# takurot/Pyrope

Hardware: NVIDIA B200
Metric: batched VEC.SEARCH QPS at fixed recall@10 (higher is better)
Workload: dtype f32 LUT / u8 codes

## Files before the change

### pyrope_b200/csrc/pq_lm.cu

```cuda
#include <cub/cub.cuh>

#include <cstdio>
#include <type_traits>

#include "common.cuh"
#include "exact_arith.cuh"
#include "kernels.h"

namespace pyrope {
namespace {

constexpr int LM_SCAN_WARPS = 8;
constexpr int LM_BUILD_WARPS = 8;
constexpr int LM_THREADS = 32 * (LM_SCAN_WARPS + LM_BUILD_WARPS);
constexpr int LM_BLK_STAGES = 6;
constexpr int LM_QS = 8;
constexpr int LM_QC = 256;
constexpr int LM_PF = 4;
constexpr int LM_HDR = 96;
constexpr int LM_MAX_DIM = 128;
constexpr int LM_LUT_BYTES = 256 * 256;
constexpr int LM_BLK_MAX = LM_HDR + LM_MAX_DIM * 32;
constexpr int LM_QSETS = 3;
constexpr int LM_SMEM = 2 * LM_LUT_BYTES + LM_BLK_STAGES * LM_BLK_MAX + LM_QSETS * LM_QS * LM_QC * 8;
constexpr float LM_QMAX = 2046.f;
constexpr float LM_QERR = 8.25f;
constexpr int LM_HB = 64;
constexpr int SEED_NQ = 2;
constexpr int SEED_CAP = 1024;
constexpr int REDO_QCAP = 2048;

struct __align__(16) LmHeader {
    int list, nvec;
    long long vbeg;
    int qid[LM_QS];
    short pslot[LM_QS];
    float s[LM_QS];
};
static_assert(LM_BUILD_WARPS == LM_QS && LM_SCAN_WARPS % 4 == 0, "one builder warp per query slot; builders start a TMEM lane quadrant");
static_assert(sizeof(LmHeader) == LM_HDR, "header size");

__device__ __forceinline__ uint32_t smem_u32(const void* p) { return (uint32_t)__cvta_generic_to_shared(p); }
__device__ __forceinline__ bool elect_one() {
    uint32_t pred;
    asm volatile("{\n\t.reg .pred p;\n\telect.sync _|p, 0xffffffff;\n\tselp.u32 %0, 1, 0, p;\n\t}" : "=r"(pred));
    return pred != 0;
}
__device__ __forceinline__ void mbar_init(uint32_t bar, uint32_t count) {
    asm volatile("mbarrier.init.shared::cta.b64 [%0], %1;" ::"r"(bar), "r"(count));
}
__device__ __forceinline__ void mbar_expect_tx(uint32_t bar, uint32_t bytes) {
    asm volatile("mbarrier.arrive.expect_tx.shared::cta.b64 _, [%0], %1;" ::"r"(bar), "r"(bytes) : "memory");
}
__device__ __forceinline__ bool mbar_try_wait(uint32_t bar, uint32_t parity) {
// ... 22 lines not shown
__device__ __forceinline__ void bulk_g2s(uint32_t dst, const void* src, uint32_t bytes, uint32_t bar) {
    asm volatile("cp.async.bulk.shared::cluster.global.mbarrier::complete_tx::bytes [%0], [%1], %2, [%3];"
                 ::"r"(dst), "l"(src), "r"(bytes), "r"(bar)
                 : "memory");
}
__device__ __forceinline__ unsigned long long pack2(float a, float b) {
    unsigned long long d;
    asm("mov.b64 %0, {%1, %2};" : "=l"(d) : "f"(a), "f"(b));
    return d;
}
__device__ __forceinline__ unsigned long long ffma2(unsigned long long a, unsigned long long b, unsigned long long c) {
    unsigned long long d;
    asm("fma.rn.f32x2 %0, %1, %2, %3;" : "=l"(d) : "l"(a), "l"(b), "l"(c));
    return d;
}



template <int N>
__device__ __forceinline__ void tmem_st(uint32_t taddr, const uint32_t (&r)[N]) {
    static_assert(N == 4 || N == 8, "4 or 8 columns");
    if (N == 8)
        asm volatile("tcgen05.st.sync.aligned.32x32b.x8.b32 [%0], {%1, %2, %3, %4, %5, %6, %7, %8};"
                     ::"r"(taddr), "r"(r[0]), "r"(r[1]), "r"(r[2]), "r"(r[3]), "r"(r[4 % N]), "r"(r[5 % N]), "r"(r[6 % N]), "r"(r[7 % N])
                     : "memory");
    else
        asm volatile("tcgen05.st.sync.aligned.32x32b.x4.b32 [%0], {%1, %2, %3, %4};"
                     ::"r"(taddr), "r"(r[0]), "r"(r[1]), "r"(r[2]), "r"(r[3])
                     : "memory");
}
template <int N>
__device__ __forceinline__ void tmem_ld(uint32_t taddr, uint32_t (&r)[N]) {
    if (N == 8)
        asm volatile("tcgen05.ld.sync.aligned.32x32b.x8.b32 {%0, %1, %2, %3, %4, %5, %6, %7}, [%8];"
                     : "=r"(r[0]), "=r"(r[1]), "=r"(r[2]), "=r"(r[3]), "=r"(r[4 % N]), "=r"(r[5 % N]), "=r"(r[6 % N]), "=r"(r[7 % N])
                     : "r"(taddr)
                     : "memory");
    else
        asm volatile("tcgen05.ld.sync.aligned.32x32b.x4.b32 {%0, %1, %2, %3}, [%4];"
                     : "=r"(r[0]), "=r"(r[1]), "=r"(r[2]), "=r"(r[3])
                     : "r"(taddr)
                     : "memory");
}
__device__ __forceinline__ void tmem_ld_wait() { asm volatile("tcgen05.wait::ld.sync.aligned;" ::: "memory"); }

struct LmParams {
    int dim, ksub, k;
    const float* codebook; const uint8_t* codes; const uint8_t* dead;
    const unsigned char* iblk; const int32_t* n_items;
    unsigned long long* pool; int32_t* pool_cnt; uint32_t* pool_thr; int pslots;
    int kc;
    uint32_t* hist;
    const float* thr0;
    const uint32_t* sinv_max;
    int2* redo; int32_t* redo_cnt;
    int32_t* item_ctr;
    const unsigned long long* thr_pub;
    unsigned long long* peer_thr[7];
    int n_peers;
// ... 76 lines not shown
    for (int w = (int)(((int64_t)blockIdx.x * blockDim.x + threadIdx.x) >> 5); w < n_items; w += wstride) {
        const int l = a.item_list[w], rel = w - a.ioff[l];
        const int64_t beg = a.list_off[l], len = a.list_off[l + 1] - beg;
        const int g = rel;
        const int pbeg = a.loff[l], pend = a.loff[l + 1];
        int qid[LM_QS], psl[LM_QS];
    #pragma unroll
        for (int j = 0; j < LM_QS; ++j) {
            const int idx = pbeg + LM_QS * g + j;
            qid[j] = idx < pend ? a.pairq[idx] : -1;
            psl[j] = idx < pend ? a.pairp[idx] : 0;
        }
        unsigned char* blkp = a.iblk + (size_t)w * a.blk;
        const int sub = a.dim >> 4, D0 = lane * 4;
        const bool on = lane * 4 < a.dim;
        const float cm = on ? __ldg(a.cmax + D0 / sub) : 0.f;
        float4 c = make_float4(0.f, 0.f, 0.f, 0.f);
        if (on) c = __ldg(reinterpret_cast<const float4*>(a.centroids + (size_t)l * a.dim) + lane);
        float scale[LM_QS];
    #pragma unroll
        for (int h = 0; h < LM_QS / 4; ++h) {
            float4 t[4];
    #pragma unroll
            for (int j = 0; j < 4; ++j) {
                float4 q = c;
                if (on && qid[4 * h + j] >= 0) q = __ldg(reinterpret_cast<const float4*>(a.Q + (size_t)qid[4 * h + j] * a.dim) + lane);
                t[j] = make_float4(-2.f * (q.x - c.x), -2.f * (q.y - c.y), -2.f * (q.z - c.z), -2.f * (q.w - c.w));
                float r2 = 0.25f * (t[j].x * t[j].x + t[j].y * t[j].y + t[j].z * t[j].z + t[j].w * t[j].w);
                if (sub == 8) r2 += __shfl_xor_sync(0xffffffffu, r2, 1);
                float b = on ? sqrtf(r2) * 1.000001f + cm : 0.f;
                b *= b;
    #pragma unroll
                for (int o = 16; o > 0; o >>= 1) b = fmaxf(b, __shfl_xor_sync(0xffffffffu, b, o));
                scale[4 * h + j] = qid[4 * h + j] >= 0 ? LM_QMAX / (b * 1.00001f + 1e-30f) : 0.f;
            }
            if (on) {
                float4* dst = reinterpret_cast<float4*>(blkp + LM_HDR + (size_t)h * a.dim * 16);
                dst[((D0 + 0) % sub) * 16 + (D0 + 0) / sub] = make_float4(t[0].x, t[1].x, t[2].x, t[3].x);
                dst[((D0 + 1) % sub) * 16 + (D0 + 1) / sub] = make_float4(t[0].y, t[1].y, t[2].y, t[3].y);
                dst[((D0 + 2) % sub) * 16 + (D0 + 2) / sub] = make_float4(t[0].z, t[1].z, t[2].z, t[3].z);
                dst[((D0 + 3) % sub) * 16 + (D0 + 3) / sub] = make_float4(t[0].w, t[1].w, t[2].w, t[3].w);
            }
        }
        if (lane == 0) {
            LmHeader h{};
            h.list = l;
            h.vbeg = beg;
            h.nvec = (int)len;
    #pragma unroll
            for (int j = 0; j < LM_QS; ++j) { h.qid[j] = qid[j]; h.pslot[j] = (short)psl[j]; h.s[j] = scale[j]; }
            *reinterpret_cast<LmHeader*>(blkp) = h;
        }
        if (lane < LM_QS) {
            float mys = 0.f;
            int myq = -1;
    #pragma unroll
// ... 133 lines not shown
            }
            if (lane == 0) {
                const float t = __uint_as_float(hi);
                const float tp = t + 2e-5f * t + 1e-5f * s_rr[warp] + 1e-12f;
                a.pool_thr[q0 + warp] = score_to_ord(-tp) - 1u;
                a.thr0[q0 + warp] = tp;
            }
        }
    }
}

template <int SUB>
__global__ void __launch_bounds__(LM_THREADS, 1) ivfpq_lm_scan_kernel(LmParams p) {
    extern __shared__ __align__(1024) unsigned char smem[];
    unsigned char* lut0 = smem;
    unsigned char* rbuf = lut0 + 2 * LM_LUT_BYTES;
    uint64_t* qkeys = reinterpret_cast<uint64_t*>(rbuf + LM_BLK_STAGES * LM_BLK_MAX);
    __shared__ __align__(8) uint64_t s_mbar[LM_BLK_STAGES + 4];
    __shared__ int s_qcnt[LM_QSETS * LM_QS];
    __shared__ int s_ti[LM_SCAN_WARPS * LM_QS];
    __shared__ float s_inv[LM_SCAN_WARPS * LM_QS];
    __shared__ uint32_t s_tmem;

    const int tid = threadIdx.x, lane = tid & 31, warp = tid >> 5;
    const bool builder = warp >= LM_SCAN_WARPS;
    const int K = p.ksub;
    const int blk = LM_HDR + p.dim * 32;
    const int n_items = *p.n_items;
    __shared__ int s_item[LM_BLK_STAGES];

    const uint32_t bar_blk = smem_u32(&s_mbar[0]);
    const uint32_t bar_full = smem_u32(&s_mbar[LM_BLK_STAGES]);
    const uint32_t bar_done = smem_u32(&s_mbar[LM_BLK_STAGES + 2]);
    if (tid == 0) {
        for (int i = 0; i < LM_BLK_STAGES; ++i) mbar_init(bar_blk + 8 * i, 1);
        for (int i = 0; i < 2; ++i) { mbar_init(bar_full + 8 * i, LM_BUILD_WARPS); mbar_init(bar_done + 8 * i, LM_SCAN_WARPS); }
        asm volatile("fence.mbarrier_init.release.cluster;" ::: "memory");
    }
    if (tid < LM_QSETS * LM_QS) s_qcnt[tid] = 0;
    for (int i = tid; i < 2 * LM_LUT_BYTES / 16; i += LM_THREADS) reinterpret_cast<uint4*>(lut0)[i] = make_uint4(0u, 0u, 0u, 0u);

    constexpr int BT = LM_BUILD_WARPS * 32;
    constexpr int EPT = 256 * 16 / BT;
    constexpr int TCOLS = (BT / 128) * EPT * SUB;
    if (warp == LM_SCAN_WARPS) {
        asm volatile("tcgen05.alloc.cta_group::1.sync.aligned.shared::cta.b32 [%0], %1;" ::"r"(smem_u32(&s_tmem)), "n"(TCOLS) : "memory");
        asm volatile("tcgen05.relinquish_alloc_permit.cta_group::1.sync.aligned;" ::: "memory");
    }
    asm volatile("tcgen05.fence::before_thread_sync;" ::: "memory");
    __syncthreads();
    asm volatile("tcgen05.fence::after_thread_sync;" ::: "memory");

    auto claim_block = [&](int i) -> bool {
        const uint32_t br = bar_blk + 8 * (i % LM_BLK_STAGES);
        const int g = atomicAdd(p.item_ctr, 1);
        if (g < n_items) {
            s_item[i % LM_BLK_STAGES] = g;
            mbar_expect_tx(br, (uint32_t)blk);
            bulk_g2s(smem_u32(rbuf + (i % LM_BLK_STAGES) * LM_BLK_MAX), p.iblk + (size_t)g * blk, (uint32_t)blk, br);
            return true;
        }
        s_item[i % LM_BLK_STAGES] = -1;
        mbar_arrive(br);
        return false;
    };

    if (builder) {
        const int bw = warp - LM_SCAN_WARPS;
        const int m = lane & 15;
        const int eb = (lane >> 4) + 2 * bw;
        const uint32_t tcb = s_tmem + ((uint32_t)((warp & 3) * 32) << 16) + (uint32_t)((bw >> 2) * EPT * SUB);
        float pn[EPT];
#pragma unroll
        for (int j = 0; j < EPT; ++j) {
            const int e = eb + (BT / 16) * j;
            float s = 0.f;
            uint32_t r[SUB];
#pragma unroll
            for (int d4 = 0; d4 < SUB / 4; ++d4) {
                float4 v = make_float4(0.f, 0.f, 0.f, 0.f);
                if (e < K) v = __ldg(reinterpret_cast<const float4*>(p.codebook + ((size_t)m * K + e) * SUB) + d4);
                r[4 * d4 + 0] = __float_as_uint(v.x); r[4 * d4 + 1] = __float_as_uint(v.y);
                r[4 * d4 + 2] = __float_as_uint(v.z); r[4 * d4 + 3] = __float_as_uint(v.w);
                s = fmaf(v.x, v.x, s); s = fmaf(v.y, v.y, s); s = fmaf(v.z, v.z, s); s = fmaf(v.w, v.w, s);
            }
            tmem_st<SUB>(tcb + j * SUB, r);
            pn[j] = s;
        }
        asm volatile("tcgen05.wait::st.sync.aligned;" ::: "memory");
        bool more = false;
        const bool claimer = bw == 0 && elect_one();
        if (claimer) more = claim_block(0);
        auto tighten = [&](int q, uint32_t ord) {
            if (p.n_peers == 0) {
                atomicMax(p.pool_thr + q, ord);
            } else if (atomicMax(p.pool_thr + q, ord) < ord) {
                const unsigned long long w = ((unsigned long long)p.epoch << 32) | ord;
                for (int r = 0; r < p.n_peers; ++r) atomicMax(p.peer_thr[r] + q, w);
            }
        };
        auto finalize = [&](const LmHeader* hd, int gitem, uint64_t* qk, int* qcnt) {
            const int j = bw;
            int* cntp = &qcnt[j];
            const int n = *cntp;
            const int q = hd->qid[j];
            if (n > 0 && q >= 0) {
                uint64_t* kq = qk + j * LM_QC;
                bool redo = n > LM_QC;
                if (!redo) {
                    const size_t ps = (size_t)q * p.pslots + hd->pslot[j];
                    unsigned long long* dst = p.pool + ps * p.kc;
                    const float err = LM_QERR / hd->s[j];
                    int kept = n;
                    float dk = 0.f;
                    if (n > p.k) {
                        const int P2 = next_pow2(n);
// ... 41 lines not shown
                                const int fl = __ffs(reach) - 1;
                                if (lane == fl) {
                                    const int bk = 2 * lane + ((cum - cc.y >= (uint32_t)p.k) ? 0 : 1);
                                    const float edge = bk == LM_HB - 1 ? t0 * 1.01f + 2.f * err : lo + wid * (float)(bk + 1);
                                    const float errq = LM_QERR * 1.001f * __uint_as_float(__ldg(p.sinv_max + q));
                                    tighten(q, score_to_ord(-(edge * 1.00001f + errq)) - 1u);
                                }
                            }
                        }
                    }
                }
                if (redo && lane == 0) p.redo[atomicAdd(p.redo_cnt, 1)] = make_int2(q, gitem * LM_QS + j);
            }
            __syncwarp();
            if (lane == 0) *cntp = 0;
        };

        auto wait_done = [&](int i) { mbar_wait(bar_done + 8 * (i & 1), (uint32_t)(i >> 1) & 1u); };
        auto hand_over = [&](int i) {
            finalize(reinterpret_cast<const LmHeader*>(rbuf + (i % LM_BLK_STAGES) * LM_BLK_MAX), s_item[i % LM_BLK_STAGES],
                     qkeys + (i % LM_QSETS) * (LM_QS * LM_QC), s_qcnt + (i % LM_QSETS) * LM_QS);
        };
        const unsigned long long magic2 = pack2(8388608.f, 8388608.f);
        const unsigned long long quarter = pack2(0.25f, 0.25f);
        int i = 0;
        for (;; ++i) {
            const int b = i & 1;
            if (i >= 2) wait_done(i - 2);
            if (more) more = claim_block(i + 1);
            mbar_wait(bar_blk + 8 * (i % LM_BLK_STAGES), (uint32_t)(i / LM_BLK_STAGES) & 1u);
            if (s_item[i % LM_BLK_STAGES] < 0) break;
            const unsigned char* blkp = rbuf + (i % LM_BLK_STAGES) * LM_BLK_MAX;
            const LmHeader* hd = reinterpret_cast<const LmHeader*>(blkp);
            if (claimer && hd->nvec > 0)
                bulk_prefetch_l2(p.codes + (size_t)hd->vbeg * 16, (uint32_t)hd->nvec * 16u);
            unsigned char* lut = lut0 + b * LM_LUT_BYTES;
#pragma unroll 1
            for (int h = 0; h < LM_QS / 4; ++h) {
                if (hd->qid[4 * h] < 0) continue;
                const ulonglong2* rt = reinterpret_cast<const ulonglong2*>(blkp + LM_HDR) + h * p.dim + m;
                unsigned long long t01[SUB], t23[SUB], rr01 = 0ull, rr23 = 0ull;
#pragma unroll
                for (int d = 0; d < SUB; ++d) {
                    const ulonglong2 v = rt[d * 16];
                    t01[d] = v.x; t23[d] = v.y;
                    rr01 = ffma2(v.x, v.x, rr01);
                    rr23 = ffma2(v.y, v.y, rr23);
                }
                const float4 sh4 = *reinterpret_cast<const float4*>(hd->s + 4 * h);
                const unsigned long long s01 = pack2(sh4.x, sh4.y), s23 = pack2(sh4.z, sh4.w);
                const bool compact = hd->qid[LM_QS / 2] < 0;
                unsigned char* lw = compact ? lut + eb * 128 + m * 8 : lut + eb * 256 + m * 16 + h * 8;
                const int jstride = compact ? (BT / 16) * 128 : (BT / 16) * 256;
                uint32_t cw[2][SUB];
                tmem_ld<SUB>(tcb, cw[0]);
                tmem_ld_wait();
#pragma unroll
                for (int j = 0; j < EPT; ++j) {
                    if (j + 1 < EPT) tmem_ld<SUB>(tcb + (j + 1) * SUB, cw[(j + 1) & 1]);
                    const unsigned long long pj = pack2(pn[j], pn[j]);
                    unsigned long long a01 = ffma2(rr01, quarter, pj), a23 = ffma2(rr23, quarter, pj);
#pragma unroll
                    for (int d = 0; d < SUB; ++d) {
                        const float c = __uint_as_float(cw[j & 1][d]);
                        const unsigned long long c2 = pack2(c, c);
                        a01 = ffma2(c2, t01[d], a01);
                        a23 = ffma2(c2, t23[d], a23);
                    }
                    a01 = ffma2(a01, s01, magic2);
                    a23 = ffma2(a23, s23, magic2);
                    const uint32_t w0 = __byte_perm((uint32_t)a01, (uint32_t)(a01 >> 32), 0x5410);
                    const uint32_t w1 = __byte_perm((uint32_t)a23, (uint32_t)(a23 >> 32), 0x5410);
                    *reinterpret_cast<uint2*>(lw + j * jstride) = make_uint2(w0, w1);
                    if (j + 1 < EPT) tmem_ld_wait();
                }
            }
            __syncwarp();
            if (lane == 0) mbar_arrive(bar_full + 8 * b);
            if (i >= 2) hand_over(i - 2);
        }
        if (i >= 2) hand_over(i - 2);
        if (i >= 1) { wait_done(i - 1); hand_over(i - 1); }
    } else {
        uint32_t op[8];
#pragma unroll
        for (int i = 0; i < 8; ++i) {
            op[i] = (uint32_t)(((lane + 2 * i) & 15) << 4) | ((uint32_t)(((lane + 2 * i + 1) & 15) << 4) << 8);
            asm volatile("" : "+r"(op[i]));
        }
        const int rot = lane & 15;

        uint4 cq[LM_PF];
        auto prefetch_item = [&](int i) -> bool {
            mbar_wait(bar_blk + 8 * (i % LM_BLK_STAGES), (uint32_t)(i / LM_BLK_STAGES) & 1u);
            if (s_item[i % LM_BLK_STAGES] < 0) return false;
            const LmHeader* h = reinterpret_cast<const LmHeader*>(rbuf + (i % LM_BLK_STAGES) * LM_BLK_MAX);
            const int nv = h->nvec;
            const uint4* cp = reinterpret_cast<const uint4*>(p.codes) + h->vbeg;
#pragma unroll
            for (int u = 0; u < LM_PF; ++u) {
                const int v = (warp + u * LM_SCAN_WARPS) * 32 + lane;
                cq[u] = make_uint4(0u, 0u, 0u, 0u);
                if (v < nv) cq[u] = __ldg(cp + v);
            }
            return true;
        };
        bool have = prefetch_item(0);
        for (int i = 0; have; ++i) {
            const int b = i & 1;
            const unsigned char* blkp = rbuf + (i % LM_BLK_STAGES) * LM_BLK_MAX;
            const LmHeader* hd = reinterpret_cast<const LmHeader*>(blkp);
            const int nvec = hd->nvec;
            const long long vbeg = hd->vbeg;
            const uint4* cp = reinterpret_cast<const uint4*>(p.codes) + vbeg;
            uint64_t* qk = qkeys + (i % LM_QSETS) * (LM_QS * LM_QC);
            int* qcnt = s_qcnt + (i % LM_QSETS) * LM_QS;
            int* ti_w = s_ti + warp * LM_QS;
            float* inv_w = s_inv + warp * LM_QS;
            {
                int ti = -1;
                float inv = 0.f;
                if (lane < LM_QS) {
                    const int myq = hd->qid[lane];
                    if (myq >= 0) {
                        const float mys = hd->s[lane];
// ... 83 lines not shown
                                    }
                                }
                            }
                        }
                    }
                }
            }
            };
            if (hd->qid[LM_QS / 2] < 0) scan_rows(std::true_type{}); else scan_rows(std::false_type{});
            have = prefetch_item(i + 1);
            __syncwarp();
            if (lane == 0) mbar_arrive(bar_done + 8 * b);
        }
    }

    asm volatile("tcgen05.fence::before_thread_sync;" ::: "memory");
    __syncthreads();
    if (warp == LM_SCAN_WARPS) {
        asm volatile("tcgen05.fence::after_thread_sync;" ::: "memory");
        asm volatile("tcgen05.dealloc.cta_group::1.sync.aligned.b32 %0, %1;" ::"r"(s_tmem), "n"(TCOLS) : "memory");
    }
}

struct LmRedo {
    const float* Q; int dim; const float* centroids; const float* codebook; int ksub;
    const uint8_t* codes; const uint8_t* dead;
    const unsigned char* iblk; int blk; const int2* redo; const int32_t* redo_cnt;
    unsigned long long* pool; int32_t* pool_cnt; int pslots; int k; int kc;
    const uint32_t* pool_thr;
};
__global__ void __launch_bounds__(256) ivfpq_lm_redo_kernel(LmRedo a) {
    extern __shared__ __align__(16) unsigned char smem_raw[];
    uint64_t* keys = reinterpret_cast<uint64_t*>(smem_raw);
    float* lut = reinterpret_cast<float*>(keys + REDO_QCAP);
    float* res = lut + 4096;
// ... 30 lines not shown
        if (tid == 0) a.pool_cnt[ps] = keep;
        for (int i = tid; i < keep; i += 256) a.pool[ps * a.kc + i] = keys[i];
    }
}

struct LmFinalParams {
    const float* Q; int dim;
    const float* centroids; const float* codebook; int ksub; int m;
    const uint8_t* codes; const int64_t* list_off; int nlist; const int64_t* labels;
    const int64_t* probes; int P; int64_t nq;
    const unsigned long long* pool; const int32_t* pool_cnt; int pslots; int k; int kc;
    const uint32_t* sinv_max;
    int keys_cap;
    PairOut out;
    int32_t* counts;
};

template <int SUB>
__global__ void __launch_bounds__(256) ivfpq_lm_final_kernel(LmFinalParams p) {
    extern __shared__ __align__(16) unsigned char smem_raw[];
    uint64_t* keys = reinterpret_cast<uint64_t*>(smem_raw);
    const int tid = threadIdx.x, lane = tid & 31, warp = tid >> 5;
    __shared__ int s_n, s_m;
    __shared__ uint32_t s_lohi[2];
    __shared__ int s_hist[256];
    __shared__ float s_lim;
    for (int64_t q = blockIdx.x; q < p.nq; q += gridDim.x) {
        if (tid == 0) { s_n = 0; s_m = 0; s_lohi[0] = 0xffffffffu; s_lohi[1] = 0u; }
        for (int i = tid; i < 256; i += blockDim.x) s_hist[i] = 0;
        __syncthreads();
// ... 60 lines not shown
            const float lim = s_lim;
            for (int i0 = 0; i0 < n; i0 += blockDim.x) {
                const int i = i0 + tid;
                const uint64_t key = i < n ? keys[i] : 0ull;
                const bool keep = i < n && -key_score(key) <= lim;
                const unsigned mk = __ballot_sync(0xffffffffu, keep);
                int base = 0;
                __syncthreads();
                if (lane == 0 && mk) base = atomicAdd(&s_m, __popc(mk));
                base = __shfl_sync(0xffffffffu, base, 0);
                if (keep) keys[base + __popc(mk & ((1u << lane) - 1u))] = key;
            }
            __syncthreads();
            nres = s_m;
        }
        const int hl = tid & 15, hw = tid >> 4, nhw = blockDim.x >> 4;
        const unsigned hmask = 0xffffu << (lane & 16);
        for (int i0 = 0; i0 < nres; i0 += nhw) {
            const int i = i0 + hw;
            const bool on = i < nres;
            const uint32_t pos = key_pos(keys[on ? i : i0]);
            int lo = 0;
            for (int p0 = 0; p0 < p.P; p0 += 16) {
                const bool hit = p0 + hl < p.P && s_lo[p0 + hl] <= (long long)pos && (long long)pos < s_hi[p0 + hl];
                const unsigned mh = __ballot_sync(0xffffffffu, hit) & hmask;
                if (mh) lo = s_list[p0 + ((__ffs(mh) - 1) & 15)];
                if (__all_sync(0xffffffffu, mh != 0 || lo != 0)) break;
            }
            float dm = 0.f, dist = 0.f;
            if (p.m == 16) {
// ... 70 lines not shown
    L.hist = o; o += align_up(sizeof(uint32_t) * (size_t)nq * LM_HB, 256);
    L.thr0 = o; o += align_up(sizeof(float) * (size_t)nq, 256);
    L.redo_cnt = o; o += 256;
    L.item_ctr = o; o += 256;
    L.scanned = o; o += 256;
    L.zero_bytes = o;
    L.cmax = o; o += 256;
    L.loff = o; o += align_up(sizeof(int32_t) * ((size_t)nlist + 1), 256);
    L.nit = o; o += align_up(sizeof(unsigned long long) * ((size_t)nlist + 2), 256);
    L.ioff = o; o += align_up(sizeof(int32_t) * ((size_t)nlist + 1), 256);
    L.pairq = o; o += align_up(sizeof(int32_t) * (size_t)npairs, 256);
    L.pairp = o; o += align_up(sizeof(int32_t) * (size_t)npairs, 256);
    L.max_items = (npairs / LM_QS + std::min<int64_t>(npairs, nlist) + 1) * maxseg;
    L.item_list = o; o += align_up(sizeof(int32_t) * (size_t)L.max_items, 256);
    L.redo = o; o += align_up(sizeof(int2) * (size_t)L.max_items * LM_QS, 256);
    L.blk = LM_HDR + dim * 32;
    L.iblk = o; o += align_up((size_t)L.blk * (size_t)L.max_items, 256);
    L.pslots = P * maxseg;
    L.kc = lm_kc(k);
    L.pool_cap = L.pslots * L.kc;
    L.pool = o; o += align_up(sizeof(unsigned long long) * (size_t)nq * L.pool_cap, 256);
    size_t tb = 0;
    {
        cub::TransformInputIterator<unsigned long long, LmPackOp, cub::CountingInputIterator<int>> it(cub::CountingInputIterator<int>(0),
                                                                                                     LmPackOp{nullptr, nlist});
        cub::DeviceScan::ExclusiveSum(nullptr, tb, it, (unsigned long long*)nullptr, nlist + 1);
    }
    L.temp_bytes = tb + 256;
    L.temp = o; o += align_up(L.temp_bytes, 256);
    L.total = o;
    return L;
// ... 107 lines not shown
    LmRedo rd{};
    rd.Q = p.Q; rd.dim = p.dim; rd.centroids = p.centroids; rd.codebook = cb16; rd.ksub = p.ksub;
    rd.codes = codes16; rd.dead = p.dead; rd.iblk = iblk; rd.blk = L.blk; rd.redo = redo; rd.redo_cnt = redo_cnt;
    rd.pool = pool; rd.pool_cnt = pool_cnt; rd.pslots = L.pslots; rd.k = p.k; rd.kc = L.kc; rd.pool_thr = pool_thr;
    const size_t redo_smem = sizeof(uint64_t) * REDO_QCAP + sizeof(float) * (4096 + (size_t)p.dim);
    mark();
    ivfpq_lm_redo_kernel<<<(unsigned)(2 * num_sms), 256, redo_smem, st>>>(rd);
    mark();

    LmFinalParams fp{};
    fp.Q = p.Q; fp.dim = p.dim; fp.centroids = p.centroids; fp.codebook = p.codebook; fp.ksub = p.ksub; fp.m = p.m;
    fp.codes = p.codes; fp.list_off = p.list_off; fp.nlist = p.nlist; fp.labels = p.labels;
    fp.probes = p.probes; fp.P = P; fp.nq = p.nq;
    fp.pool = pool; fp.pool_cnt = pool_cnt; fp.pslots = L.pslots; fp.k = p.k; fp.kc = L.kc; fp.sinv_max = sinv_max; fp.out = p.out; fp.counts = p.out_counts;
    fp.keys_cap = next_pow2(std::max(2, L.pool_cap));
    const int fthreads = L.pool_cap <= 2048 ? 128 : 256;
    const size_t fsm = sizeof(uint64_t) * (size_t)fp.keys_cap + (2 * sizeof(long long) + sizeof(int)) * (size_t)P +
                       (p.m == 16 ? 0 : sizeof(float) * (size_t)(fthreads / 16) * p.dim);
    e = cudaFuncSetAttribute(ivfpq_lm_final_kernel<SUB>, cudaFuncAttributeMaxDynamicSharedMemorySize, (int)fsm);
    if (e != cudaSuccess) return e;
    ivfpq_lm_final_kernel<SUB><<<(unsigned)p.nq, fthreads, fsm, st>>>(fp);
    mark();
    if (stage_dbg && nsev == 7) {
        cudaEventSynchronize(sev[6]);
        const char* names[6] = {"group", "prepare", "seed", "scan", "redo", "final"};
        fprintf(stderr, "[lm stages]");
        for (int i = 0; i < 6; ++i) {
            float ms = 0.f;
            cudaEventElapsedTime(&ms, sev[i], sev[i + 1]);
            fprintf(stderr, " %s=%.3fms", names[i], ms);
        }
        int nredo = 0;
        cudaMemcpy(&nredo, redo_cnt, sizeof(int), cudaMemcpyDeviceToHost);
        int nitems = 0;
        cudaMemcpy(&nitems, ioff + p.nlist, sizeof(int), cudaMemcpyDeviceToHost);
        fprintf(stderr, " items=%d redo=%d\n", nitems, nredo);
        for (int i = 0; i < nsev; ++i) cudaEventDestroy(sev[i]);
    }
    return cudaGetLastError();
}

__global__ void lm_expand_codebook_kernel(const float* __restrict__ cb, int m, int ksub, int dim, float* __restrict__ cb16) {
    const int sub16 = dim / 16, subr = dim / m, per = 16 / m;
    const int64_t n = (int64_t)16 * ksub * sub16;
    for (int64_t i = (int64_t)blockIdx.x * blockDim.x + threadIdx.x; i < n; i += (int64_t)gridDim.x * blockDim.x) {
        const int d = (int)(i % sub16), e = (int)((i / sub16) % ksub), v = (int)(i / ((int64_t)sub16 * ksub));
        cb16[i] = cb[((size_t)(v / per) * ksub + e) * subr + (v % per) * sub16 + d];
    }
}
__global__ void lm_expand_codes_kernel(const uint8_t* __restrict__ codes, int64_t n, int m, uint4* __restrict__ codes16) {
    const int per = 16 / m;
// ... 56 lines not shown
```

Measured before the change: 2.210 million.

## Build per-item PQ LUTs with tcgen05 TF32 MMA instead of scalar FMA

Measured after the change: 1.802 million, median of 6. 0.815x the previous value.

```diff
diff --git a/pyrope_b200/csrc/pq_lm.cu b/pyrope_b200/csrc/pq_lm.cu
--- a/pyrope_b200/csrc/pq_lm.cu
+++ b/pyrope_b200/csrc/pq_lm.cu
@@ -18,13 +18,17 @@
 constexpr int LM_QC = 256;
 constexpr int LM_PF = 4;
 constexpr int LM_HDR = 96;
-constexpr int LM_MAX_DIM = 128;
+constexpr int LM_BTAB = 256;
+constexpr int LM_RR = LM_HDR + 16 * LM_BTAB;
+constexpr int LM_BLK = LM_RR + 16 * LM_QS * 4;
 constexpr int LM_LUT_BYTES = 256 * 256;
-constexpr int LM_BLK_MAX = LM_HDR + LM_MAX_DIM * 32;
+constexpr int LM_ZB = 256;
 constexpr int LM_QSETS = 3;
-constexpr int LM_SMEM = 2 * LM_LUT_BYTES + LM_BLK_STAGES * LM_BLK_MAX + LM_QSETS * LM_QS * LM_QC * 8;
+constexpr int LM_SMEM = 2 * LM_LUT_BYTES + 2 * LM_ZB + LM_BLK_STAGES * LM_BLK + LM_QSETS * LM_QS * LM_QC * 8;
+constexpr int LM_TCOLS = 512;
+constexpr int LM_TACC = 256;
 constexpr float LM_QMAX = 2046.f;
-constexpr float LM_QERR = 8.25f;
+constexpr float LM_QERR = 24.5f;
 constexpr int LM_HB = 64;
 constexpr int SEED_NQ = 2;
 constexpr int SEED_CAP = 1024;
@@ -37,7 +41,8 @@
     short pslot[LM_QS];
     float s[LM_QS];
 };
-static_assert(LM_BUILD_WARPS == LM_QS && LM_SCAN_WARPS % 4 == 0, "one builder warp per query slot; builders start a TMEM lane quadrant");
+static_assert(LM_BUILD_WARPS == 8 && LM_BUILD_WARPS == LM_QS && LM_SCAN_WARPS % 4 == 0,
+              "builder warp w reads TMEM lane quadrant w % 4 (code half w / 4) and hands over slot w");
 static_assert(sizeof(LmHeader) == LM_HDR, "header size");
 
 __device__ __forceinline__ uint32_t smem_u32(const void* p) { return (uint32_t)__cvta_generic_to_shared(p); }
@@ -90,35 +95,52 @@
     asm("fma.rn.f32x2 %0, %1, %2, %3;" : "=l"(d) : "l"(a), "l"(b), "l"(c));
     return d;
 }
-
-
-
-template <int N>
-__device__ __forceinline__ void tmem_st(uint32_t taddr, const uint32_t (&r)[N]) {
-    static_assert(N == 4 || N == 8, "4 or 8 columns");
-    if (N == 8)
-        asm volatile("tcgen05.st.sync.aligned.32x32b.x8.b32 [%0], {%1, %2, %3, %4, %5, %6, %7, %8};"
-                     ::"r"(taddr), "r"(r[0]), "r"(r[1]), "r"(r[2]), "r"(r[3]), "r"(r[4 % N]), "r"(r[5 % N]), "r"(r[6 % N]), "r"(r[7 % N])
-                     : "memory");
-    else
-        asm volatile("tcgen05.st.sync.aligned.32x32b.x4.b32 [%0], {%1, %2, %3, %4};"
-                     ::"r"(taddr), "r"(r[0]), "r"(r[1]), "r"(r[2]), "r"(r[3])
-                     : "memory");
-}
-template <int N>
-__device__ __forceinline__ void tmem_ld(uint32_t taddr, uint32_t (&r)[N]) {
-    if (N == 8)
-        asm volatile("tcgen05.ld.sync.aligned.32x32b.x8.b32 {%0, %1, %2, %3, %4, %5, %6, %7}, [%8];"
-                     : "=r"(r[0]), "=r"(r[1]), "=r"(r[2]), "=r"(r[3]), "=r"(r[4 % N]), "=r"(r[5 % N]), "=r"(r[6 % N]), "=r"(r[7 % N])
-                     : "r"(taddr)
-                     : "memory");
-    else
-        asm volatile("tcgen05.ld.sync.aligned.32x32b.x4.b32 {%0, %1, %2, %3}, [%4];"
-                     : "=r"(r[0]), "=r"(r[1]), "=r"(r[2]), "=r"(r[3])
-                     : "r"(taddr)
-                     : "memory");
+__device__ __forceinline__ unsigned long long fadd2(unsigned long long a, unsigned long long b) {
+    unsigned long long d;
+    asm("add.rn.f32x2 %0, %1, %2;" : "=l"(d) : "l"(a), "l"(b));
+    return d;
+}
+__device__ __forceinline__ uint32_t to_tf32(float x) {
+    uint32_t r;
+    asm("cvt.rna.tf32.f32 %0, %1;" : "=r"(r) : "f"(x));
+    return r;
+}
+
+__device__ __forceinline__ void tmem_st8(uint32_t taddr, const uint32_t (&r)[8]) {
+    asm volatile("tcgen05.st.sync.aligned.32x32b.x8.b32 [%0], {%1, %2, %3, %4, %5, %6, %7, %8};"
+                 ::"r"(taddr), "r"(r[0]), "r"(r[1]), "r"(r[2]), "r"(r[3]), "r"(r[4]), "r"(r[5]), "r"(r[6]), "r"(r[7])
+                 : "memory");
+}
+__device__ __forceinline__ void tmem_ld16(uint32_t taddr, uint32_t (&r)[16]) {
+    asm volatile("tcgen05.ld.sync.aligned.32x32b.x16.b32 {%0, %1, %2, %3, %4, %5, %6, %7, %8, %9, %10, %11, %12, %13, %14, %15}, [%16];"
+                 : "=r"(r[0]), "=r"(r[1]), "=r"(r[2]), "=r"(r[3]), "=r"(r[4]), "=r"(r[5]), "=r"(r[6]), "=r"(r[7]),
+                   "=r"(r[8]), "=r"(r[9]), "=r"(r[10]), "=r"(r[11]), "=r"(r[12]), "=r"(r[13]), "=r"(r[14]), "=r"(r[15])
+                 : "r"(taddr)
+                 : "memory");
 }
 __device__ __forceinline__ void tmem_ld_wait() { asm volatile("tcgen05.wait::ld.sync.aligned;" ::: "memory"); }
+__device__ __forceinline__ void tc_fence_before() { asm volatile("tcgen05.fence::before_thread_sync;" ::: "memory"); }
+__device__ __forceinline__ void tc_fence_after() { asm volatile("tcgen05.fence::after_thread_sync;" ::: "memory"); }
+__device__ __forceinline__ uint64_t make_kmajor_desc(uint32_t saddr, uint32_t lbo, uint32_t sbo) {
+    uint64_t d = 0;
+    d |= (uint64_t)((saddr & 0x3FFFFu) >> 4);
+    d |= (uint64_t)((lbo & 0x3FFFFu) >> 4) << 16;
+    d |= (uint64_t)((sbo & 0x3FFFFu) >> 4) << 32;
+    d |= (uint64_t)1 << 46;
+    return d;
+}
+constexpr uint32_t LM_IDESC = (1u << 4) | (2u << 7) | (2u << 10) | ((uint32_t)(16 >> 3) << 17) | ((uint32_t)(128 >> 4) << 24);
+__device__ __forceinline__ void mma_tf32_ts(uint32_t tmem_d, uint32_t tmem_a, uint64_t bdesc, uint32_t accum) {
+    asm volatile(
+        "{\n\t.reg .pred p;\n\tsetp.ne.b32 p, %3, 0;\n\t"
+        "tcgen05.mma.cta_group::1.kind::tf32 [%0], [%1], %2, %4, p;\n\t}"
+        ::"r"(tmem_d), "r"(tmem_a), "l"(bdesc), "r"(accum), "r"(LM_IDESC)
+        : "memory");
+}
+__device__ __forceinline__ void tc_commit(uint32_t bar) {
+    asm volatile("tcgen05.commit.cta_group::1.mbarrier::arrive::one.shared::cluster.b64 [%0];" ::"r"(bar) : "memory");
+}
+__device__ __forceinline__ void builders_sync() { asm volatile("bar.sync 1, %0;" ::"n"(32 * LM_BUILD_WARPS) : "memory"); }
 
 struct LmParams {
     int dim, ksub, k;
@@ -225,32 +247,29 @@
         unsigned char* blkp = a.iblk + (size_t)w * a.blk;
         const int sub = a.dim >> 4, D0 = lane * 4;
         const bool on = lane * 4 < a.dim;
-        const float cm = on ? __ldg(a.cmax + D0 / sub) : 0.f;
+        const int mi = on ? D0 / sub : 0, kb = (D0 % sub) >> 2;
+        const float cm = on ? __ldg(a.cmax + mi) : 0.f;
         float4 c = make_float4(0.f, 0.f, 0.f, 0.f);
         if (on) c = __ldg(reinterpret_cast<const float4*>(a.centroids + (size_t)l * a.dim) + lane);
         float scale[LM_QS];
+        unsigned char* bt = blkp + LM_HDR + mi * LM_BTAB + kb * 128;
+        float* rrp = reinterpret_cast<float*>(blkp + LM_RR) + mi * LM_QS;
     #pragma unroll
-        for (int h = 0; h < LM_QS / 4; ++h) {
-            float4 t[4];
+        for (int j = 0; j < LM_QS; ++j) {
+            float4 q = c;
+            if (on && qid[j] >= 0) q = __ldg(reinterpret_cast<const float4*>(a.Q + (size_t)qid[j] * a.dim) + lane);
+            const float4 t = make_float4(-2.f * (q.x - c.x), -2.f * (q.y - c.y), -2.f * (q.z - c.z), -2.f * (q.w - c.w));
+            float r2 = 0.25f * (t.x * t.x + t.y * t.y + t.z * t.z + t.w * t.w);
+            if (sub == 8) r2 += __shfl_xor_sync(0xffffffffu, r2, 1);
+            float b = on ? sqrtf(r2) * 1.000001f + cm : 0.f;
+            b *= b;
     #pragma unroll
-            for (int j = 0; j < 4; ++j) {
-                float4 q = c;
-                if (on && qid[4 * h + j] >= 0) q = __ldg(reinterpret_cast<const float4*>(a.Q + (size_t)qid[4 * h + j] * a.dim) + lane);
-                t[j] = make_float4(-2.f * (q.x - c.x), -2.f * (q.y - c.y), -2.f * (q.z - c.z), -2.f * (q.w - c.w));
-                float r2 = 0.25f * (t[j].x * t[j].x + t[j].y * t[j].y + t[j].z * t[j].z + t[j].w * t[j].w);
-                if (sub == 8) r2 += __shfl_xor_sync(0xffffffffu, r2, 1);
-                float b = on ? sqrtf(r2) * 1.000001f + cm : 0.f;
-                b *= b;
-    #pragma unroll
-                for (int o = 16; o > 0; o >>= 1) b = fmaxf(b, __shfl_xor_sync(0xffffffffu, b, o));
-                scale[4 * h + j] = qid[4 * h + j] >= 0 ? LM_QMAX / (b * 1.00001f + 1e-30f) : 0.f;
-            }
+            for (int o = 16; o > 0; o >>= 1) b = fmaxf(b, __shfl_xor_sync(0xffffffffu, b, o));
+            scale[j] = qid[j] >= 0 ? LM_QMAX / (b * 1.00001f + 1e-30f) : 0.f;
             if (on) {
-                float4* dst = reinterpret_cast<float4*>(blkp + LM_HDR + (size_t)h * a.dim * 16);
-                dst[((D0 + 0) % sub) * 16 + (D0 + 0) / sub] = make_float4(t[0].x, t[1].x, t[2].x, t[3].x);
-                dst[((D0 + 1) % sub) * 16 + (D0 + 1) / sub] = make_float4(t[0].y, t[1].y, t[2].y, t[3].y);
-                dst[((D0 + 2) % sub) * 16 + (D0 + 2) / sub] = make_float4(t[0].z, t[1].z, t[2].z, t[3].z);
-                dst[((D0 + 3) % sub) * 16 + (D0 + 3) / sub] = make_float4(t[0].w, t[1].w, t[2].w, t[3].w);
+                *reinterpret_cast<uint4*>(bt + j * 16) = make_uint4(to_tf32(t.x), to_tf32(t.y), to_tf32(t.z), to_tf32(t.w));
+                if (sub == 4) *reinterpret_cast<uint4*>(bt + 128 + j * 16) = make_uint4(0u, 0u, 0u, 0u);
+                if (kb == 0) rrp[j] = r2;
             }
         }
         if (lane == 0) {
@@ -414,9 +433,11 @@
 __global__ void __launch_bounds__(LM_THREADS, 1) ivfpq_lm_scan_kernel(LmParams p) {
     extern __shared__ __align__(1024) unsigned char smem[];
     unsigned char* lut0 = smem;
-    unsigned char* rbuf = lut0 + 2 * LM_LUT_BYTES;
-    uint64_t* qkeys = reinterpret_cast<uint64_t*>(rbuf + LM_BLK_STAGES * LM_BLK_MAX);
-    __shared__ __align__(8) uint64_t s_mbar[LM_BLK_STAGES + 4];
+    unsigned char* zlo = lut0 + 2 * LM_LUT_BYTES;
+    unsigned char* rbuf = zlo + LM_ZB;
+    unsigned char* zhi = rbuf + LM_BLK_STAGES * LM_BLK;
+    uint64_t* qkeys = reinterpret_cast<uint64_t*>(zhi + LM_ZB);
+    __shared__ __align__(8) uint64_t s_mbar[LM_BLK_STAGES + 5];
     __shared__ int s_qcnt[LM_QSETS * LM_QS];
     __shared__ int s_ti[LM_SCAN_WARPS * LM_QS];
     __shared__ float s_inv[LM_SCAN_WARPS * LM_QS];
@@ -425,39 +446,42 @@
     const int tid = threadIdx.x, lane = tid & 31, warp = tid >> 5;
     const bool builder = warp >= LM_SCAN_WARPS;
     const int K = p.ksub;
-    const int blk = LM_HDR + p.dim * 32;
     const int n_items = *p.n_items;
     __shared__ int s_item[LM_BLK_STAGES];
 
     const uint32_t bar_blk = smem_u32(&s_mbar[0]);
     const uint32_t bar_full = smem_u32(&s_mbar[LM_BLK_STAGES]);
     const uint32_t bar_done = smem_u32(&s_mbar[LM_BLK_STAGES + 2]);
+    const uint32_t bar_mma = smem_u32(&s_mbar[LM_BLK_STAGES + 4]);
     if (tid == 0) {
         for (int i = 0; i < LM_BLK_STAGES; ++i) mbar_init(bar_blk + 8 * i, 1);
         for (int i = 0; i < 2; ++i) { mbar_init(bar_full + 8 * i, LM_BUILD_WARPS); mbar_init(bar_done + 8 * i, LM_SCAN_WARPS); }
+        mbar_init(bar_mma, 1);
         asm volatile("fence.mbarrier_init.release.cluster;" ::: "memory");
     }
     if (tid < LM_QSETS * LM_QS) s_qcnt[tid] = 0;
     for (int i = tid; i < 2 * LM_LUT_BYTES / 16; i += LM_THREADS) reinterpret_cast<uint4*>(lut0)[i] = make_uint4(0u, 0u, 0u, 0u);
-
-    constexpr int BT = LM_BUILD_WARPS * 32;
-    constexpr int EPT = 256 * 16 / BT;
-    constexpr int TCOLS = (BT / 128) * EPT * SUB;
+    for (int i = tid; i < LM_ZB / 16; i += LM_THREADS) {
+        reinterpret_cast<uint4*>(zlo)[i] = make_uint4(0u, 0u, 0u, 0u);
+        reinterpret_cast<uint4*>(zhi)[i] = make_uint4(0u, 0u, 0u, 0u);
+    }
+    asm volatile("fence.proxy.async.shared::cta;" ::: "memory");
+
     if (warp == LM_SCAN_WARPS) {
-        asm volatile("tcgen05.alloc.cta_group::1.sync.aligned.shared::cta.b32 [%0], %1;" ::"r"(smem_u32(&s_tmem)), "n"(TCOLS) : "memory");
+        asm volatile("tcgen05.alloc.cta_group::1.sync.aligned.shared::cta.b32 [%0], %1;" ::"r"(smem_u32(&s_tmem)), "n"(LM_TCOLS) : "memory");
         asm volatile("tcgen05.relinquish_alloc_permit.cta_group::1.sync.aligned;" ::: "memory");
     }
-    asm volatile("tcgen05.fence::before_thread_sync;" ::: "memory");
+    tc_fence_before();
     __syncthreads();
-    asm volatile("tcgen05.fence::after_thread_sync;" ::: "memory");
+    tc_fence_after();
 
     auto claim_block = [&](int i) -> bool {
         const uint32_t br = bar_blk + 8 * (i % LM_BLK_STAGES);
         const int g = atomicAdd(p.item_ctr, 1);
         if (g < n_items) {
             s_item[i % LM_BLK_STAGES] = g;
-            mbar_expect_tx(br, (uint32_t)blk);
-            bulk_g2s(smem_u32(rbuf + (i % LM_BLK_STAGES) * LM_BLK_MAX), p.iblk + (size_t)g * blk, (uint32_t)blk, br);
+            mbar_expect_tx(br, (uint32_t)LM_BLK);
+            bulk_g2s(smem_u32(rbuf + (i % LM_BLK_STAGES) * LM_BLK), p.iblk + (size_t)g * LM_BLK, (uint32_t)LM_BLK, br);
             return true;
         }
         s_item[i % LM_BLK_STAGES] = -1;
@@ -467,25 +491,27 @@
 
     if (builder) {
         const int bw = warp - LM_SCAN_WARPS;
-        const int m = lane & 15;
-        const int eb = (lane >> 4) + 2 * bw;
-        const uint32_t tcb = s_tmem + ((uint32_t)((warp & 3) * 32) << 16) + (uint32_t)((bw >> 2) * EPT * SUB);
-        float pn[EPT];
-#pragma unroll
-        for (int j = 0; j < EPT; ++j) {
-            const int e = eb + (BT / 16) * j;
-            float s = 0.f;
-            uint32_t r[SUB];
-#pragma unroll
-            for (int d4 = 0; d4 < SUB / 4; ++d4) {
-                float4 v = make_float4(0.f, 0.f, 0.f, 0.f);
-                if (e < K) v = __ldg(reinterpret_cast<const float4*>(p.codebook + ((size_t)m * K + e) * SUB) + d4);
-                r[4 * d4 + 0] = __float_as_uint(v.x); r[4 * d4 + 1] = __float_as_uint(v.y);
-                r[4 * d4 + 2] = __float_as_uint(v.z); r[4 * d4 + 3] = __float_as_uint(v.w);
-                s = fmaf(v.x, v.x, s); s = fmaf(v.y, v.y, s); s = fmaf(v.z, v.z, s); s = fmaf(v.w, v.w, s);
-            }
-            tmem_st<SUB>(tcb + j * SUB, r);
-            pn[j] = s;
+        const int quad = warp & 3;
+        const int half = bw >> 2;
+        const int e = half * 128 + quad * 32 + lane;
+        const uint32_t tq = s_tmem + ((uint32_t)(quad * 32) << 16);
+        float pn[16];
+        {
+#pragma unroll
+            for (int m = 0; m < 16; ++m) {
+                float s = 0.f;
+                uint32_t r[8];
+#pragma unroll
+                for (int d4 = 0; d4 < 2; ++d4) {
+                    float4 v = make_float4(0.f, 0.f, 0.f, 0.f);
+                    if (e < K && d4 < SUB / 4) v = __ldg(reinterpret_cast<const float4*>(p.codebook + ((size_t)m * K + e) * SUB) + d4);
+                    r[4 * d4 + 0] = to_tf32(v.x); r[4 * d4 + 1] = to_tf32(v.y);
+                    r[4 * d4 + 2] = to_tf32(v.z); r[4 * d4 + 3] = to_tf32(v.w);
+                    s = fmaf(v.x, v.x, s); s = fmaf(v.y, v.y, s); s = fmaf(v.z, v.z, s); s = fmaf(v.w, v.w, s);
+                }
+                tmem_st8(tq + (uint32_t)((half * 16 + m) * 8), r);
+                pn[m] = s;
+            }
         }
         asm volatile("tcgen05.wait::st.sync.aligned;" ::: "memory");
         bool more = false;
@@ -500,6 +526,7 @@
             }
         };
         auto finalize = [&](const LmHeader* hd, int gitem, uint64_t* qk, int* qcnt) {
+          {
             const int j = bw;
             int* cntp = &qcnt[j];
             const int n = *cntp;
@@ -571,15 +598,91 @@
             }
             __syncwarp();
             if (lane == 0) *cntp = 0;
+          }
         };
 
         auto wait_done = [&](int i) { mbar_wait(bar_done + 8 * (i & 1), (uint32_t)(i >> 1) & 1u); };
         auto hand_over = [&](int i) {
-            finalize(reinterpret_cast<const LmHeader*>(rbuf + (i % LM_BLK_STAGES) * LM_BLK_MAX), s_item[i % LM_BLK_STAGES],
+            finalize(reinterpret_cast<const LmHeader*>(rbuf + (i % LM_BLK_STAGES) * LM_BLK), s_item[i % LM_BLK_STAGES],
                      qkeys + (i % LM_QSETS) * (LM_QS * LM_QC), s_qcnt + (i % LM_QSETS) * LM_QS);
         };
         const unsigned long long magic2 = pack2(8388608.f, 8388608.f);
-        const unsigned long long quarter = pack2(0.25f, 0.25f);
+        auto build = [&](auto nw_tag, const unsigned char* blkp, const LmHeader* hd, unsigned char* lut) {
+            constexpr int NW = decltype(nw_tag)::value;
+            constexpr int G = 32 / NW;
+            unsigned long long s2[NW];
+#pragma unroll
+            for (int w = 0; w < NW; ++w) s2[w] = pack2(hd->s[2 * w], hd->s[2 * w + 1]);
+            const float* rrp = reinterpret_cast<const float*>(blkp + LM_RR);
+#pragma unroll
+            for (int g0 = 0; g0 < 16; g0 += G) {
+                uint32_t W[G][NW];
+#pragma unroll
+                for (int u0 = 0; u0 < G / 2; u0 += 2) {
+                    uint32_t v[2][16];
+                    tmem_ld16(tq + (uint32_t)(LM_TACC + (half * 8 + g0 / 2 + u0) * 16), v[0]);
+                    tmem_ld16(tq + (uint32_t)(LM_TACC + (half * 8 + g0 / 2 + u0 + 1) * 16), v[1]);
+                    tmem_ld_wait();
+#pragma unroll
+                    for (int x = 0; x < 4; ++x) {
+                        const int m = g0 + 2 * u0 + x;
+                        const unsigned long long pj = pack2(pn[m], pn[m]);
+                        float rq[2 * NW];
+#pragma unroll
+                        for (int w = 0; w < NW / 2; ++w) {
+                            const float4 r4 = *reinterpret_cast<const float4*>(rrp + m * LM_QS + 4 * w);
+                            rq[4 * w] = r4.x; rq[4 * w + 1] = r4.y; rq[4 * w + 2] = r4.z; rq[4 * w + 3] = r4.w;
+                        }
+#pragma unroll
+                        for (int w = 0; w < NW; ++w) {
+                            const unsigned long long c = fadd2(pack2(rq[2 * w], rq[2 * w + 1]), pj);
+                            const uint32_t* vv = v[x >> 1] + 8 * (x & 1) + 2 * w;
+                            const unsigned long long tv = fadd2(pack2(__uint_as_float(vv[0]), __uint_as_float(vv[1])), c);
+                            const unsigned long long q = ffma2(tv, s2[w], magic2);
+                            W[2 * u0 + x][w] = __vmaxs2(__byte_perm((uint32_t)q, (uint32_t)(q >> 32), 0x5410), 0u);
+                        }
+                    }
+                }
+#pragma unroll
+                for (int bit = 1; bit < G; bit <<= 1) {
+                    const bool sh = lane & bit;
+                    uint32_t X[G][NW];
+#pragma unroll
+                    for (int g = 0; g < G; ++g) {
+#pragma unroll
+                        for (int w = 0; w < NW; ++w) X[g][w] = sh ? W[(g + bit) % G][w] : W[g][w];
+                    }
+#pragma unroll
+                    for (int g = 0; g < G; ++g) {
+#pragma unroll
+                        for (int w = 0; w < NW; ++w) W[g][w] = X[g][w];
+                    }
+                }
+#pragma unroll
+                for (int g = 0; g < G; ++g) {
+                    const int m = g0 + ((g + lane) & (G - 1));
+                    if (NW == 4)
+                        *reinterpret_cast<uint4*>(lut + e * 256 + m * 16) = make_uint4(W[g][0], W[g][1], W[g][2 % NW], W[g][3 % NW]);
+                    else
+                        *reinterpret_cast<uint2*>(lut + e * 128 + m * 8) = make_uint2(W[g][0], W[g][1]);
+                }
+            }
+        };
+        auto issue_products = [&](int i) {
+            const uint32_t bt = smem_u32(rbuf + (i % LM_BLK_STAGES) * LM_BLK + LM_HDR), z0 = smem_u32(zlo), z1 = smem_u32(zhi);
+#pragma unroll 1
+            for (int h = 0; h < 2; ++h) {
+#pragma unroll
+                for (int u = 0; u < 8; ++u) {
+                    const uint32_t d = s_tmem + (uint32_t)(LM_TACC + (h * 8 + u) * 16);
+                    const uint32_t a0 = s_tmem + (uint32_t)((h * 16 + 2 * u) * 8);
+                    const uint32_t b0 = bt + (uint32_t)(2 * u * LM_BTAB), b1 = b0 + LM_BTAB;
+                    mma_tf32_ts(d, a0, make_kmajor_desc(b0, 128, z1 - b0), 0u);
+                    mma_tf32_ts(d, a0 + 8, make_kmajor_desc(z0, 128, b1 - z0), 1u);
+                }
+            }
+            tc_commit(bar_mma);
+        };
         int i = 0;
         for (;; ++i) {
             const int b = i & 1;
@@ -587,53 +690,32 @@
             if (more) more = claim_block(i + 1);
             mbar_wait(bar_blk + 8 * (i % LM_BLK_STAGES), (uint32_t)(i / LM_BLK_STAGES) & 1u);
             if (s_item[i % LM_BLK_STAGES] < 0) break;
-            const unsigned char* blkp = rbuf + (i % LM_BLK_STAGES) * LM_BLK_MAX;
+            const unsigned char* blkp = rbuf + (i % LM_BLK_STAGES) * LM_BLK;
             const LmHeader* hd = reinterpret_cast<const LmHeader*>(blkp);
             if (claimer && hd->nvec > 0)
                 bulk_prefetch_l2(p.codes + (size_t)hd->vbeg * 16, (uint32_t)hd->nvec * 16u);
+            if (i == 0) {
+                tc_fence_before();
+                builders_sync();
+                tc_fence_after();
+                if (bw == 0 && elect_one()) issue_products(0);
+                __syncwarp();
+            }
+            mbar_wait(bar_mma, (uint32_t)i & 1u);
+            tc_fence_after();
             unsigned char* lut = lut0 + b * LM_LUT_BYTES;
-#pragma unroll 1
-            for (int h = 0; h < LM_QS / 4; ++h) {
-                if (hd->qid[4 * h] < 0) continue;
-                const ulonglong2* rt = reinterpret_cast<const ulonglong2*>(blkp + LM_HDR) + h * p.dim + m;
-                unsigned long long t01[SUB], t23[SUB], rr01 = 0ull, rr23 = 0ull;
-#pragma unroll
-                for (int d = 0; d < SUB; ++d) {
-                    const ulonglong2 v = rt[d * 16];
-                    t01[d] = v.x; t23[d] = v.y;
-                    rr01 = ffma2(v.x, v.x, rr01);
-                    rr23 = ffma2(v.y, v.y, rr23);
-                }
-                const float4 sh4 = *reinterpret_cast<const float4*>(hd->s + 4 * h);
-                const unsigned long long s01 = pack2(sh4.x, sh4.y), s23 = pack2(sh4.z, sh4.w);
-                const bool compact = hd->qid[LM_QS / 2] < 0;
-                unsigned char* lw = compact ? lut + eb * 128 + m * 8 : lut + eb * 256 + m * 16 + h * 8;
-                const int jstride = compact ? (BT / 16) * 128 : (BT / 16) * 256;
-                uint32_t cw[2][SUB];
-                tmem_ld<SUB>(tcb, cw[0]);
-                tmem_ld_wait();
-#pragma unroll
-                for (int j = 0; j < EPT; ++j) {
-                    if (j + 1 < EPT) tmem_ld<SUB>(tcb + (j + 1) * SUB, cw[(j + 1) & 1]);
-                    const unsigned long long pj = pack2(pn[j], pn[j]);
-                    unsigned long long a01 = ffma2(rr01, quarter, pj), a23 = ffma2(rr23, quarter, pj);
-#pragma unroll
-                    for (int d = 0; d < SUB; ++d) {
-                        const float c = __uint_as_float(cw[j & 1][d]);
-                        const unsigned long long c2 = pack2(c, c);
-                        a01 = ffma2(c2, t01[d], a01);
-                        a23 = ffma2(c2, t23[d], a23);
-                    }
-                    a01 = ffma2(a01, s01, magic2);
-                    a23 = ffma2(a23, s23, magic2);
-                    const uint32_t w0 = __byte_perm((uint32_t)a01, (uint32_t)(a01 >> 32), 0x5410);
-                    const uint32_t w1 = __byte_perm((uint32_t)a23, (uint32_t)(a23 >> 32), 0x5410);
-                    *reinterpret_cast<uint2*>(lw + j * jstride) = make_uint2(w0, w1);
-                    if (j + 1 < EPT) tmem_ld_wait();
-                }
-            }
+            if (hd->qid[LM_QS / 2] < 0) build(std::integral_constant<int, 2>{}, blkp, hd, lut);
+            else build(std::integral_constant<int, 4>{}, blkp, hd, lut);
             __syncwarp();
             if (lane == 0) mbar_arrive(bar_full + 8 * b);
+            tc_fence_before();
+            builders_sync();
+            tc_fence_after();
+            if (bw == 0 && elect_one()) {
+                mbar_wait(bar_blk + 8 * ((i + 1) % LM_BLK_STAGES), (uint32_t)((i + 1) / LM_BLK_STAGES) & 1u);
+                if (s_item[(i + 1) % LM_BLK_STAGES] >= 0) issue_products(i + 1);
+            }
+            __syncwarp();
             if (i >= 2) hand_over(i - 2);
         }
         if (i >= 2) hand_over(i - 2);
@@ -651,7 +733,7 @@
         auto prefetch_item = [&](int i) -> bool {
             mbar_wait(bar_blk + 8 * (i % LM_BLK_STAGES), (uint32_t)(i / LM_BLK_STAGES) & 1u);
             if (s_item[i % LM_BLK_STAGES] < 0) return false;
-            const LmHeader* h = reinterpret_cast<const LmHeader*>(rbuf + (i % LM_BLK_STAGES) * LM_BLK_MAX);
+            const LmHeader* h = reinterpret_cast<const LmHeader*>(rbuf + (i % LM_BLK_STAGES) * LM_BLK);
             const int nv = h->nvec;
             const uint4* cp = reinterpret_cast<const uint4*>(p.codes) + h->vbeg;
 #pragma unroll
@@ -665,7 +747,7 @@
         bool have = prefetch_item(0);
         for (int i = 0; have; ++i) {
             const int b = i & 1;
-            const unsigned char* blkp = rbuf + (i % LM_BLK_STAGES) * LM_BLK_MAX;
+            const unsigned char* blkp = rbuf + (i % LM_BLK_STAGES) * LM_BLK;
             const LmHeader* hd = reinterpret_cast<const LmHeader*>(blkp);
             const int nvec = hd->nvec;
             const long long vbeg = hd->vbeg;
@@ -779,11 +861,11 @@
         }
     }
 
-    asm volatile("tcgen05.fence::before_thread_sync;" ::: "memory");
+    tc_fence_before();
     __syncthreads();
     if (warp == LM_SCAN_WARPS) {
-        asm volatile("tcgen05.fence::after_thread_sync;" ::: "memory");
-        asm volatile("tcgen05.dealloc.cta_group::1.sync.aligned.b32 %0, %1;" ::"r"(s_tmem), "n"(TCOLS) : "memory");
+        tc_fence_after();
+        asm volatile("tcgen05.dealloc.cta_group::1.sync.aligned.b32 %0, %1;" ::"r"(s_tmem), "n"(LM_TCOLS) : "memory");
     }
 }
 
@@ -844,6 +926,7 @@
     int keys_cap;
     PairOut out;
     int32_t* counts;
+    int32_t* n_rescored;
 };
 
 template <int SUB>
@@ -934,6 +1017,7 @@
             __syncthreads();
             nres = s_m;
         }
+        if (p.n_rescored && tid == 0) atomicAdd(p.n_rescored, nres);
         const int hl = tid & 15, hw = tid >> 4, nhw = blockDim.x >> 4;
         const unsigned hmask = 0xffffu << (lane & 16);
         for (int i0 = 0; i0 < nres; i0 += nhw) {
@@ -1034,7 +1118,7 @@
     L.max_items = (npairs / LM_QS + std::min<int64_t>(npairs, nlist) + 1) * maxseg;
     L.item_list = o; o += align_up(sizeof(int32_t) * (size_t)L.max_items, 256);
     L.redo = o; o += align_up(sizeof(int2) * (size_t)L.max_items * LM_QS, 256);
-    L.blk = LM_HDR + dim * 32;
+    L.blk = LM_BLK;
     L.iblk = o; o += align_up((size_t)L.blk * (size_t)L.max_items, 256);
     L.pslots = P * maxseg;
     L.kc = lm_kc(k);
@@ -1172,6 +1256,10 @@
     fp.probes = p.probes; fp.P = P; fp.nq = p.nq;
     fp.pool = pool; fp.pool_cnt = pool_cnt; fp.pslots = L.pslots; fp.k = p.k; fp.kc = L.kc; fp.sinv_max = sinv_max; fp.out = p.out; fp.counts = p.out_counts;
     fp.keys_cap = next_pow2(std::max(2, L.pool_cap));
+    if (stage_dbg) {
+        fp.n_rescored = reinterpret_cast<int32_t*>(base + L.item_ctr);
+        cudaMemsetAsync(fp.n_rescored, 0, sizeof(int32_t), st);
+    }
     const int fthreads = L.pool_cap <= 2048 ? 128 : 256;
     const size_t fsm = sizeof(uint64_t) * (size_t)fp.keys_cap + (2 * sizeof(long long) + sizeof(int)) * (size_t)P +
                        (p.m == 16 ? 0 : sizeof(float) * (size_t)(fthreads / 16) * p.dim);
@@ -1192,7 +1280,9 @@
         cudaMemcpy(&nredo, redo_cnt, sizeof(int), cudaMemcpyDeviceToHost);
         int nitems = 0;
         cudaMemcpy(&nitems, ioff + p.nlist, sizeof(int), cudaMemcpyDeviceToHost);
-        fprintf(stderr, " items=%d redo=%d\n", nitems, nredo);
+        int nres = 0;
+        cudaMemcpy(&nres, base + L.item_ctr, sizeof(int), cudaMemcpyDeviceToHost);
+        fprintf(stderr, " items=%d redo=%d rescored=%d\n", nitems, nredo, nres);
         for (int i = 0; i < nsev; ++i) cudaEventDestroy(sev[i]);
     }
     return cudaGetLastError();
```
